# chanchanchan97/ICAFusion

Measured on AMD Instinct MI355X. Metric: RGB/IR image-pairs/sec (two-stream forward + NMS), higher is better.
Workload: dtype bf16

## Files before the change

icafusion_amd/csrc/conv_common.h:

```cpp
#pragma once
#include "icaf_common.h"

namespace icaf {

struct ConvP {
    const void* x; const void* w; const float* bias; void* y; const void* res;
    long long x_gs, w_gs, bias_gs, y_gs, res_gs;
    int B, H, W, Cin, ldx, Ho, Wo, Cout, ldy, kh, kw, sh, sw, ph, pw, ldr, Kp, act;
    int M, K, nchunks, mtiles, ntiles;
    int vec_y, vec_r;
    unsigned int x_bytes, w_bytes;
    float alpha_acc[2], alpha_res[2];
    const float* pre; int pre_h, pre_w, ldpre, pre_mode;
    const void* w1; const float* bias1;
    long long w1_gs, bias1_gs; int Kp1; unsigned int w1_bytes;
    const void* w2; const float* bias2; void* y2;
    long long w2_gs, bias2_gs, y2_gs; int Kp2, Cout2, ldy2, vec_y2, keep1; unsigned int w2_bytes;
    const void* x2; long long x2_gs; int ldx2;
};

constexpr int ROWB = 64;
constexpr int ROWS = 80;
constexpr int NTHREADS = 256;

int ctile_conv_check(const icaf_conv_args* a, const ConvP& p, int shape);
int launch_ctile(const icaf_conv_args* a, const ConvP& p, int shape, hipStream_t s);
const char* ctile_tag(int shape);
int stream_check(const icaf_conv_args* a, const ConvP& p, int shape);
int launch_stream(const icaf_conv_args* a, const ConvP& p, int shape, hipStream_t s);
const char* stream_tag(int shape);
int wreg_check(const icaf_conv_args* a, const ConvP& p, int shape);
int launch_wreg(const icaf_conv_args* a, const ConvP& p, int shape, hipStream_t s);
const char* wreg_tag(int shape);
int cstream_check(const icaf_conv_args* a, const ConvP& p, int shape);
int launch_cstream(const icaf_conv_args* a, const ConvP& p, int shape, hipStream_t s);
const char* cstream_tag(int shape);
int cwide_check(const icaf_conv_args* a, const ConvP& p, int shape);
int launch_cwide(const icaf_conv_args* a, const ConvP& p, int shape, hipStream_t s);
const char* cwide_tag(int shape);
int launch_bneck(const icaf_conv_args* a, const ConvP& p, int shape, hipStream_t s);

constexpr int ACT_RELU_RES = 16 + ICAF_ACT_RELU;
template <int ACT, int DT = ICAF_F32> __device__ __forceinline__ float apply_act(float v) {
    if constexpr (ACT == ICAF_ACT_SILU) return silu_f(v);
    else if constexpr (ACT == ICAF_ACT_GELU) return DT == ICAF_F32 ? gelu_f(v) : gelu_fast_f(v);
    else if constexpr (ACT == ICAF_ACT_RELU || ACT == ACT_RELU_RES) return fmaxf(v, 0.0f);
    else return v;
}
template <int DT> __device__ __forceinline__ void load_res_quad(const typename Elem<DT>::type* __restrict__ rg, int m, int ldr, int n, int Cout, int vec_r, float (&r)[4]) {
    using E = Elem<DT>;
#pragma unroll
    for (int j = 0; j < 4; ++j) r[j] = 0.0f;
    if (m < 0 || n >= Cout) return;
    const typename E::type* rp = rg + (long long)m * ldr + n;
    if (vec_r && n + 4 <= Cout) {
        if constexpr (DT == ICAF_F32) {
            const f32x4 t = *(const f32x4*)rp;
#pragma unroll
            for (int j = 0; j < 4; ++j) r[j] = t[j];
        } else {
            const u32x2 t = *(const u32x2*)rp;
            if constexpr (DT == ICAF_BF16) {
                r[0] = __uint_as_float(t[0] << 16); r[1] = __uint_as_float(t[0] & 0xffff0000u);
                r[2] = __uint_as_float(t[1] << 16); r[3] = __uint_as_float(t[1] & 0xffff0000u);
            } else {
                r[0] = f16_to_f32((unsigned short)(t[0] & 0xffffu)); r[1] = f16_to_f32((unsigned short)(t[0] >> 16));
                r[2] = f16_to_f32((unsigned short)(t[1] & 0xffffu)); r[3] = f16_to_f32((unsigned short)(t[1] >> 16));
            }
        }
    } else {
        for (int j = 0; j < 4 && n + j < Cout; ++j) r[j] = E::ld(rp + j);
    }
}
template <int ACT, int DT = ICAF_F32> __device__ __forceinline__ void apply_act4(const float (&x)[4], float (&y)[4]) {
    if constexpr (ACT == ICAF_ACT_SILU) silu4_f(x, y);
    else {
#pragma unroll
        for (int j = 0; j < 4; ++j) y[j] = apply_act<ACT, DT>(x[j]);
    }
}

__device__ __forceinline__ int xcd_tile(int ntile_total) {
    const int bid = blockIdx.x, q = ntile_total >> 3, r = ntile_total & 7, xcd = bid & 7, idx = bid >> 3;
    return (xcd < r ? xcd * (q + 1) : r * (q + 1) + (xcd - r) * q) + idx;
}

template <int DT, int ODT, int BM, int BN, int WM, int WN, int ACT, bool PRE, bool SECOND = false, bool WB = false, bool FULLVEC = false, typename RowMap>
__device__ __forceinline__ void epilogue(f32x16 (&acc)[WN / 32][WM / 32], unsigned char* lds, const ConvP& p, int g, RowMap row_to_m, int n0) {
    using E = Elem<DT>;
    using EO = Elem<ODT>;
    constexpr int TM = WM / 32, TN = WN / 32;
    constexpr int WAVES_M = BM / WM;
    constexpr int NT = (BM / WM) * (BN / WN) * 64;
    constexpr int VO = 16 / EO::BYTES;
    constexpr int SO = BN * EO::BYTES + 16;
    const int tid = threadIdx.x, lane = tid & 63, wave = tid >> 6, l31 = lane & 31, hi = lane >> 5;
    const int wm = wave % WAVES_M, wn = wave / WAVES_M;
    const float alpha_acc = SECOND ? 1.0f : p.alpha_acc[g], alpha_res = p.alpha_res[g];
    const float* __restrict__ bias = SECOND ? (p.bias2 ? p.bias2 + g * p.bias2_gs : nullptr) : (p.bias ? p.bias + g * p.bias_gs : nullptr);
    const int Cout = SECOND ? p.Cout2 : p.Cout, ldy = SECOND ? p.ldy2 : p.ldy, vec_y = SECOND ? p.vec_y2 : p.vec_y;
    static_assert(ACT != ACT_RELU_RES || (!PRE && !SECOND && !WB && !FULLVEC && ODT == DT), "res_mode = 1: a plain same-type layer");
    if constexpr (PRE) {
        constexpr int SOF = BN * 4 + 16;
#pragma unroll
        for (int a = 0; a < TN; ++a) {
            f32x4 bq[4];
#pragma unroll
            for (int q = 0; q < 4; ++q) {
                const int n = n0 + wn * WN + a * 32 + 8 * q + 4 * hi;
                const bool okn = bias && n < Cout;
                const float* bp = okn ? bias + n : (const float*)p.w;
                const f32x4 t = *(const f32x4*)bp;
                bq[q] = okn ? t : f32x4{0.f, 0.f, 0.f, 0.f};
            }
#pragma unroll
            for (int q = 0; q < 4; ++q) {
                const int nl = wn * WN + a * 32 + 8 * q + 4 * hi;
#pragma unroll
                for (int b = 0; b < TM; ++b) {
                    const int ml = wm * WM + b * 32 + l31;
                    f32x4 t;
#pragma unroll
                    for (int j = 0; j < 4; ++j) t[j] = acc[a][b][4 * q + j] + bq[q][j];
                    *(f32x4*)(lds + ml * SOF + nl * 4) = t;
                }
            }
        }
        __syncthreads();
        typename EO::type* __restrict__ yg2 = SECOND ? (typename EO::type*)p.y2 + g * p.y2_gs : (typename EO::type*)p.y + g * p.y_gs;
        const typename E::type* __restrict__ rg2 = (!SECOND && p.res) ? (const typename E::type*)p.res + g * p.res_gs : nullptr;
        constexpr int VPR2 = BN / VO, NVEC2 = BM * VPR2, NIT2 = (NVEC2 + NT - 1) / NT;
        const float sy = (float)p.pre_h / (float)p.Ho, sx = (float)p.pre_w / (float)p.Wo;
#pragma unroll 2
        for (int it = 0; it < NIT2; ++it) {
            const int idx = tid + it * NT;
            if (idx >= NVEC2) break;
            const int row = idx / VPR2, cv = idx - row * VPR2;
            const int m = row_to_m(row), n = n0 + cv * VO;
            if (m < 0 || n >= Cout) continue;
            const float* pt4[4];
            float lx, ly;
            {
#pragma clang fp contract(off)
                const int wo = m % p.Wo, t = m / p.Wo, ho = t % p.Ho, bi = t / p.Ho;
                float fy = ((float)ho + 0.5f) * sy - 0.5f, fx = ((float)wo + 0.5f) * sx - 0.5f;
                fy = fy < 0.0f ? 0.0f : fy;
                fx = fx < 0.0f ? 0.0f : fx;
                int y0 = (int)fy, x0 = (int)fx;
                y0 = y0 < p.pre_h - 1 ? y0 : p.pre_h - 1;
                x0 = x0 < p.pre_w - 1 ? x0 : p.pre_w - 1;
                int y1 = y0 < p.pre_h - 1 ? y0 + 1 : y0, x1 = x0 < p.pre_w - 1 ? x0 + 1 : x0;
                ly = fy - (float)y0;
                lx = fx - (float)x0;
                if (p.pre_mode == 1) {
                    y0 = y1 = (int)((long long)ho * p.pre_h / p.Ho);
                    x0 = x1 = (int)((long long)wo * p.pre_w / p.Wo);
                    ly = lx = 0.0f;
                }
                const float* base = p.pre + (long long)bi * p.pre_h * p.pre_w * p.ldpre + n;
                pt4[0] = base + (long long)(y0 * p.pre_w + x0) * p.ldpre;
                pt4[1] = base + (long long)(y0 * p.pre_w + x1) * p.ldpre;
                pt4[2] = base + (long long)(y1 * p.pre_w + x0) * p.ldpre;
                pt4[3] = base + (long long)(y1 * p.pre_w + x1) * p.ldpre;
            }
            const int nvalid = (Cout - n) < VO ? (Cout - n) : VO;
            float v[VO];
#pragma unroll
            for (int k4 = 0; k4 < VO / 4; ++k4) {
                const f32x4 t = *(const f32x4*)(lds + row * SOF + (cv * VO + 4 * k4) * 4);
                float pv[4] = {0.f, 0.f, 0.f, 0.f};
                if (n + 4 * k4 < Cout) {
                    const f32x4 t00 = *(const f32x4*)(pt4[0] + 4 * k4), t01 = *(const f32x4*)(pt4[1] + 4 * k4);
                    const f32x4 t10 = *(const f32x4*)(pt4[2] + 4 * k4), t11 = *(const f32x4*)(pt4[3] + 4 * k4);
                    {
#pragma clang fp contract(off)
                        const float wx0 = 1.0f - lx, wy0 = 1.0f - ly;
#pragma unroll
                        for (int j = 0; j < 4; ++j) {
                            const float top = t00[j] * wx0 + t01[j] * lx;
                            const float bot = t10[j] * wx0 + t11[j] * lx;
                            pv[j] = top * wy0 + bot * ly;
                        }
                    }
                }
#pragma unroll
                for (int j = 0; j < 4; ++j) v[4 * k4 + j] = apply_act<ACT, DT>(t[j] + pv[j]) * alpha_acc;
            }
            u32x4 o = pack16<ODT>(v);
            typename EO::type* yp = yg2 + (long long)m * ldy + n;
            if (rg2) {
                unpack16<ODT>(o, v);
                const typename E::type* rp = rg2 + (long long)m * p.ldr + n;
                for (int j = 0; j < nvalid; ++j) v[j] = __builtin_fmaf(alpha_res, E::ld(rp + j), v[j]);
                o = pack16<ODT>(v);
            }
            if (vec_y && nvalid == VO) *(u32x4*)yp = o;
            else {
                unpack16<ODT>(o, v);
                for (int j = 0; j < nvalid; ++j) EO::st(yp + j, v[j]);
            }
        }
        return;
    }
#pragma unroll
    for (int a = 0; a < TN; ++a) {
        f32x4 bq[4];
#pragma unroll
        for (int q = 0; q < 4; ++q) {
            const int n = n0 + wn * WN + a * 32 + 8 * q + 4 * hi;
            const bool okn = bias && n < Cout;
            const float* bp = okn ? bias + n : (const float*)p.w;
            const f32x4 t = *(const f32x4*)bp;
            bq[q] = okn ? t : f32x4{0.f, 0.f, 0.f, 0.f};
        }
#pragma unroll
        for (int q = 0; q < 4; ++q) {
            const int nl = wn * WN + a * 32 + 8 * q + 4 * hi;
            const float bv[4] = {bq[q][0], bq[q][1], bq[q][2], bq[q][3]};
#pragma unroll
            for (int b = 0; b < TM; ++b) {
                const int ml = wm * WM + b * 32 + l31;
                float v[4], xin[4];
#pragma unroll
                for (int j = 0; j < 4; ++j) xin[j] = acc[a][b][4 * q + j] + bv[j] + 0.0f;
                if constexpr (ACT == ACT_RELU_RES) {
                    float rq[4];
                    load_res_quad<DT>((const typename E::type*)p.res + g * p.res_gs, row_to_m(ml), p.ldr, n0 + nl, Cout, p.vec_r, rq);
#pragma unroll
                    for (int j = 0; j < 4; ++j) xin[j] += rq[j];
                }
                apply_act4<ACT, DT>(xin, v);
#pragma unroll
                for (int j = 0; j < 4; ++j) v[j] *= alpha_acc;
                unsigned char* dst = lds + ml * SO + nl * EO::BYTES;
                if constexpr (EO::BYTES == 4) {
                    *(f32x4*)dst = f32x4{v[0], v[1], v[2], v[3]};
                } else {
                    u32x2 pk;
                    if constexpr (ODT == ICAF_BF16) { pk[0] = pack2_bf16(v[0], v[1]); pk[1] = pack2_bf16(v[2], v[3]); }
                    else { pk[0] = pack2_f16(v[0], v[1]); pk[1] = pack2_f16(v[2], v[3]); }
                    *(u32x2*)dst = pk;
                }
            }
        }
    }
    __syncthreads();

    typename EO::type* __restrict__ yg = SECOND ? (typename EO::type*)p.y2 + g * p.y2_gs : (typename EO::type*)p.y + g * p.y_gs;
    const typename E::type* __restrict__ rg = (!SECOND && p.res && ACT != ACT_RELU_RES) ? (const typename E::type*)p.res + g * p.res_gs : nullptr;
    constexpr int VPR = BN / VO;
    constexpr int NVEC = BM * VPR;
    constexpr int NIT = (NVEC + NT - 1) / NT;
    if constexpr (FULLVEC) {
        static_assert(!WB && NVEC % NT == 0 && (VPR & (VPR - 1)) == 0, "whole rounds of power-of-two rows");
#pragma unroll
        for (int it = 0; it < NIT; ++it) {
            const int idx = tid + it * NT, row = idx / VPR, cv = idx & (VPR - 1);
            const int m = row_to_m(row);
            if (m >= 0) *(u32x4*)(yg + (long long)m * ldy + n0 + cv * VO) = *(const u32x4*)(lds + row * SO + cv * 16);
        }
        return;
    }
    if constexpr (VO == E::VEC && NVEC % NT == 0 && (VPR & (VPR - 1)) == 0) {
        if (vec_y && n0 + BN <= Cout && (!rg || p.vec_r)) {
            if (!rg) {
#pragma unroll
                for (int it = 0; it < NIT; ++it) {
                    const int idx = tid + it * NT, row = idx / VPR, cv = idx & (VPR - 1);
                    const int m = row_to_m(row);
// ... 174 lines not shown
```

icafusion_amd/csrc/dmff.hip:

```cpp
#include <cstdlib>
#include "icaf_common.h"
#include "attn_core.h"

namespace icaf {

static inline unsigned grid_for(long long total) {
    long long b = (total + 255) / 256;
    if (b > 256 * 16) b = 256 * 16;
    if (b < 1) b = 1;
    return (unsigned)b;
}

struct PoolDiv { FastDiv nv, N, tw; };
template <int DT, bool I32>
__global__ __launch_bounds__(256) void pool_tokens_kernel(const typename Elem<DT>::type* __restrict__ f0, int ld0,
                                                          const typename Elem<DT>::type* __restrict__ f1, int ld1,
                                                          const float* __restrict__ pos0, const float* __restrict__ pos1,
                                                          typename Elem<DT>::type* __restrict__ tok, int B, int H, int W, int C, int th,
                                                          int tw, int kh, int kw, int sh, int sw, float w1_0, float w2_0, float w1_1,
                                                          float w2_1, PoolDiv dv) {
    using E = Elem<DT>;
    const int nv = C / E::VEC, N = th * tw;
    const long long per_g = (long long)B * N * nv, total = 2 * per_g;
    const float inv_area = 1.0f / (float)(kh * kw);
    for (long long idx = (long long)blockIdx.x * blockDim.x + threadIdx.x; idx < total; idx += (long long)gridDim.x * blockDim.x) {
        const int g = idx >= per_g;
        const long long r = idx - (g ? per_g : 0);
        int v, n, b, oy, ox;
        if constexpr (I32) {
            unsigned int bn, uv, un, ub, uoy, uox;
            fd_divmod((unsigned int)r, dv.nv, bn, uv);
            fd_divmod(bn, dv.N, ub, un);
            fd_divmod(un, dv.tw, uoy, uox);
            v = (int)uv; n = (int)un; b = (int)ub; oy = (int)uoy; ox = (int)uox;
        } else {
            v = (int)(r % nv);
            const long long bn = r / nv;
            n = (int)(bn % N); b = (int)(bn / N);
            oy = n / tw; ox = n - oy * tw;
        }
        const typename E::type* f = g ? f1 : f0;
        const int ld = g ? ld1 : ld0;
        float sum[E::VEC], mx[E::VEC];
#pragma unroll
        for (int j = 0; j < E::VEC; ++j) { sum[j] = 0.0f; mx[j] = -INFINITY; }
        const typename E::type* f00 = f + (((long long)b * H + oy * sh) * W + ox * sw) * ld + v * E::VEC;
        for (int dy = 0; dy < kh; ++dy) {
            const typename E::type* frow = f00 + (long long)dy * W * ld;
            for (int dx0 = 0; dx0 < kw; dx0 += 4) {
                u32x4 raw[4];
#pragma unroll
                for (int u = 0; u < 4; ++u)
                    if (dx0 + u < kw) raw[u] = *(const u32x4*)(frow + (long long)(dx0 + u) * ld);
#pragma unroll
                for (int u = 0; u < 4; ++u) {
                    if (dx0 + u < kw) {
                        float t[E::VEC];
                        unpack16<DT>(raw[u], t);
#pragma unroll
                        for (int j = 0; j < E::VEC; ++j) { sum[j] += t[j]; mx[j] = fmaxf(mx[j], t[j]); }
                    }
                }
            }
        }
        const float w1 = g ? w1_1 : w1_0, w2 = g ? w2_1 : w2_0;
        const float* pos = (g ? pos1 : pos0) + (long long)n * C + v * E::VEC;
        float o[E::VEC];
#pragma unroll
        for (int j = 0; j < E::VEC; ++j) o[j] = (sum[j] * inv_area) * w1 + mx[j] * w2 + pos[j];
        *(u32x4*)(tok + (((long long)g * B + b) * N + n) * C + v * E::VEC) = pack16<DT>(o);
    }
}

template <int DT, int R, int TR>
__global__ __launch_bounds__(1024) void pool_tokens_rows_kernel(const typename Elem<DT>::type* __restrict__ f0, int ld0,
                                                                const typename Elem<DT>::type* __restrict__ f1, int ld1,
                                                                const float* __restrict__ pos0, const float* __restrict__ pos1,
                                                                typename Elem<DT>::type* __restrict__ tok, int B, int H, int W, int C,
                                                                int th, int tw, int kh, int kw, int sh, int sw, float w1_0, float w2_0,
                                                                float w1_1, float w2_1) {
    using E = Elem<DT>;
    constexpr int V = E::VEC;
    extern __shared__ __attribute__((aligned(16))) unsigned char lds_raw[];
    const int nv = C / V, nitem = W * nv;
    float* csum = (float*)lds_raw;
    u32x4* cmax = (u32x4*)(csum + (size_t)TR * nitem * V);
    const int nblk = gridDim.x, bid = blockIdx.x;
    const int qd = nblk >> 3, rm = nblk & 7, xcd = bid & 7, ix = bid >> 3;
    const int row = (xcd < rm ? xcd * (qd + 1) : rm * (qd + 1) + (xcd - rm) * qd) + ix;
    const int thb = (th + TR - 1) / TR;
    const int g = row / (B * thb), r = row - g * (B * thb), b = r / thb, oy0 = (r - b * thb) * TR;
    const int ntr = th - oy0 < TR ? th - oy0 : TR;
    const int nrow = kh + (ntr - 1) * sh;
    const typename E::type* f = g ? f1 : f0;
    const int ld = g ? ld1 : ld0;
    const typename E::type* frow = f + ((long long)b * H + oy0 * sh) * W * ld;
    const long long rstride = (long long)W * ld;
    for (int item = threadIdx.x; item < nitem; item += blockDim.x) {
        const int x = item / nv, v = item - x * nv;
        const typename E::type* p0 = frow + (long long)x * ld + v * V;
        float sum[TR][V], mx[TR][V];
#pragma unroll
        for (int t = 0; t < TR; ++t)
#pragma unroll
            for (int j = 0; j < V; ++j) { sum[t][j] = 0.0f; mx[t][j] = -INFINITY; }
        for (int d0 = 0; d0 < nrow; d0 += R) {
            u32x4 raw[R];
#pragma unroll
            for (int u = 0; u < R; ++u) {
                const int d = d0 + u < nrow ? d0 + u : nrow - 1;
                raw[u] = *(const u32x4*)(p0 + d * rstride);
            }
#pragma unroll
            for (int u = 0; u < R; ++u) {
                float t[V];
                unpack16<DT>(raw[u], t);
#pragma unroll
                for (int k = 0; k < TR; ++k) {
                    const int dd = d0 + u - k * sh;
                    if (dd >= 0 && dd < kh && k < ntr) {
                        asm volatile("");
#pragma unroll
                        for (int j = 0; j < V; ++j) {
                            sum[k][j] += t[j];
                            mx[k][j] = fmaxf(mx[k][j], t[j]);
                        }
                    }
                }
            }
        }
#pragma unroll
        for (int k = 0; k < TR; ++k) {
#pragma unroll
            for (int j = 0; j < V; j += 4)
                *(f32x4*)(csum + ((size_t)k * nitem + item) * V + j) = f32x4{sum[k][j], sum[k][j + 1], sum[k][j + 2], sum[k][j + 3]};
            cmax[(size_t)k * nitem + item] = pack16<DT>(mx[k]);
        }
    }
    __syncthreads();
    const float inv_area = 1.0f / (float)(kh * kw);
    const float w1 = g ? w1_1 : w1_0, w2 = g ? w2_1 : w2_0;
    const int N = th * tw, per = tw * nv;
    for (int o = threadIdx.x; o < ntr * per; o += blockDim.x) {
        const int k = o / per, o1 = o - k * per, ox = o1 / nv, v = o1 - ox * nv;
        float sum[V], mx[V];
#pragma unroll
        for (int j = 0; j < V; ++j) { sum[j] = 0.0f; mx[j] = -INFINITY; }
        for (int dx = 0; dx < kw; ++dx) {
            const size_t it = (size_t)k * nitem + (size_t)(ox * sw + dx) * nv + v;
            float m[V];
            unpack16<DT>(cmax[it], m);
#pragma unroll
            for (int j = 0; j < V; j += 4) {
                const f32x4 a = *(const f32x4*)(csum + it * V + j);
#pragma unroll
                for (int e = 0; e < 4; ++e) { sum[j + e] += a[e]; mx[j + e] = fmaxf(mx[j + e], m[j + e]); }
            }
        }
        const int n = (oy0 + k) * tw + ox;
        const float* pos = (g ? pos1 : pos0) + (long long)n * C + v * V;
        float out[V];
#pragma unroll
        for (int j = 0; j < V; ++j) out[j] = (sum[j] * inv_area) * w1 + mx[j] * w2 + pos[j];
        *(u32x4*)(tok + (((long long)g * B + b) * N + n) * C + v * V) = pack16<DT>(out);
    }
}

template <int DT>
__global__ __launch_bounds__(256) void layernorm_kernel(const typename Elem<DT>::type* __restrict__ x, typename Elem<DT>::type* __restrict__ y,
                                                        const float* __restrict__ g0, const float* __restrict__ b0,
                                                        const float* __restrict__ g1, const float* __restrict__ b1,
                                                        long long rows_per_group, int C, int groups, float eps) {
    using E = Elem<DT>;
    constexpr int MAXV = 4;
    const int lane = threadIdx.x & 63;
    const long long row = (long long)blockIdx.x * (blockDim.x >> 6) + (threadIdx.x >> 6);
    if (row >= rows_per_group * groups) return;
    const int grp = (int)(row / rows_per_group);
    const float* gam = grp ? g1 : g0;
    const float* bet = grp ? b1 : b0;
    const int nv = C / E::VEC;
    float val[MAXV][E::VEC];
    float s = 0.0f;
#pragma unroll
    for (int i = 0; i < MAXV; ++i) {
        const int v = lane + 64 * i;
        if (v < nv) {
            unpack16<DT>(*(const u32x4*)(x + row * C + v * E::VEC), val[i]);
#pragma unroll
            for (int j = 0; j < E::VEC; ++j) s += val[i][j];
        }
    }
#pragma unroll
    for (int o = 32; o > 0; o >>= 1) s += __shfl_xor(s, o);
    const float mean = s / (float)C;
    float q = 0.0f;
#pragma unroll
    for (int i = 0; i < MAXV; ++i) {
        const int v = lane + 64 * i;
        if (v < nv) {
#pragma unroll
            for (int j = 0; j < E::VEC; ++j) { const float d = val[i][j] - mean; q += d * d; }
        }
    }
#pragma unroll
    for (int o = 32; o > 0; o >>= 1) q += __shfl_xor(q, o);
    const float rstd = 1.0f / sqrtf(q / (float)C + eps);
#pragma unroll
    for (int i = 0; i < MAXV; ++i) {
        const int v = lane + 64 * i;
        if (v < nv) {
            float o[E::VEC];
#pragma unroll
            for (int j = 0; j < E::VEC; ++j) o[j] = (val[i][j] - mean) * rstd * gam[v * E::VEC + j] + bet[v * E::VEC + j];
            *(u32x4*)(y + row * C + v * E::VEC) = pack16<DT>(o);
        }
    }
}

template <int DT, int MAXV>
__device__ __forceinline__ void layernorm_row(const typename Elem<DT>::type* __restrict__ x, typename Elem<DT>::type* __restrict__ y,
                                              const float* __restrict__ g0, const float* __restrict__ b0,
                                              const float* __restrict__ g1, const float* __restrict__ b1,
                                              long long rows_per_group, int C, int groups, float eps) {
    using E = Elem<DT>;
    const int lane = threadIdx.x & 63;
    const long long row = (long long)blockIdx.x * (blockDim.x >> 6) + (threadIdx.x >> 6);
    if (row >= rows_per_group * groups) return;
    const int grp = (int)(row / rows_per_group);
    const float* gam = grp ? g1 : g0;
    const float* bet = grp ? b1 : b0;
    const int nv = C / E::VEC;
    float val[MAXV][E::VEC];
    float s = 0.0f;
#pragma unroll
    for (int i = 0; i < MAXV; ++i) {
        const int v = lane + 64 * i;
        if (v < nv) {
            unpack16<DT>(*(const u32x4*)(x + row * C + v * E::VEC), val[i]);
#pragma unroll
            for (int j = 0; j < E::VEC; ++j) s += val[i][j];
        }
    }
#pragma unroll
    for (int o = 32; o > 0; o >>= 1) s += __shfl_xor(s, o);
    const float mean = s / (float)C;
// ... 490 lines not shown
    ICAF_HIP(hipGetDevice(&dev));
    if (lds > 64 * 1024 && dev >= 0 && dev < ICAF_MAX_DEVICES && !attr_set[dev]) {
        ICAF_HIP(hipFuncSetAttribute((const void*)cross_attn_kernel<DT, DKP>, hipFuncAttributeMaxDynamicSharedMemorySize, 160 * 1024));
        attr_set[dev] = true;
    }
    const float scale_l2e = (float)((1.0 / sqrt((double)DK)) * 1.4426950408889634);
    dim3 grid((unsigned)qsplit, (unsigned)heads, (unsigned)(2 * B));
    if (c.remap) grid = dim3((unsigned)(qsplit * heads * 2 * B), 1u, 1u);
    hipLaunchKernelGGL((cross_attn_kernel<DT, DKP>), grid, dim3(256), lds, s, (const T*)qkv, (T*)out, B, N, C, DK, NP, scale_l2e, c.remap ? qsplit : 0);
    ICAF_LAUNCH_CHECK();
    return ICAF_OK;
}

template <int DT>
static int dispatch_attn(const void* qkv, void* out, int B, int N, int C, int heads, const AttnCfg& c, hipStream_t s) {
    switch (c.dkp) {
        case 16: return launch_attn<DT, 16>(qkv, out, B, N, C, heads, c, s);
        case 32: return launch_attn<DT, 32>(qkv, out, B, N, C, heads, c, s);
        case 48: return launch_attn<DT, 48>(qkv, out, B, N, C, heads, c, s);
        case 64: return launch_attn<DT, 64>(qkv, out, B, N, C, heads, c, s);
        case 96: return launch_attn<DT, 96>(qkv, out, B, N, C, heads, c, s);
        default: return launch_attn<DT, 128>(qkv, out, B, N, C, heads, c, s);
    }
}

struct PoolCfg { int kernel, R, TR, index64; size_t row_lds; };

static int pool_select(int dtype, int B, int H, int W, int C, int th, int tw, int kh, int kw, int sh, int sw, PoolCfg& c) {
    if (dtype < ICAF_F32 || dtype > ICAF_F16) return fail(ICAF_ERR_ARG, "bad dtype %d", dtype);
    const int vec = dtype == ICAF_F32 ? 4 : 8;
    if (C < 1 || C % vec) return fail(ICAF_ERR_ARG, "icaf_dmff_pool_tokens: C/ld must be multiples of %d", vec);
    if (B < 1 || th < 1 || tw < 1 || sh < 1 || sw < 1) return fail(ICAF_ERR_ARG, "icaf_dmff_pool_tokens: bad B / token grid / stride");
    if ((th - 1) * sh + kh > H || (tw - 1) * sw + kw > W || kh < 1 || kw < 1) return fail(ICAF_ERR_ARG, "icaf_dmff_pool_tokens: window exceeds the feature map");
    c.row_lds = (size_t)W * (C / vec) * (vec * sizeof(float) + 16);
    c.kernel = 0; c.R = 0; c.TR = 0; c.index64 = 0;
    if ((kh > sh || kw > sw) && c.row_lds <= 160 * 1024) {
        c.TR = (2 * c.row_lds <= 160 * 1024 && kh > sh && kh + sh <= 12 && 2 * B * ((th + 1) / 2) >= 256) ? 2 : 1;
        const int nrow = kh + (c.TR - 1) * sh;
        c.R = nrow <= 4 ? 4 : nrow <= 8 ? 8 : 12;
        c.kernel = 1;
        return ICAF_OK;
    }
    const long long total = 2LL * B * th * tw * (C / vec);
    c.index64 = total >= (1ll << 31) || g_opt.index64 != 0;
    return ICAF_OK;
}

}

using namespace icaf;

namespace {
template <int DT>
int run_pool_tokens(const void* f0, int ld0, const void* f1, int ld1, const float* p0, const float* p1, void* tok, int B, int H, int W, int C,
                    int th, int tw, int kh, int kw, int sh, int sw, float a0, float b0, float a1, float b1, const PoolCfg& c, hipStream_t s) {
    using T = typename Elem<DT>::type;
    if (c.kernel == 1) {
        const int tr = c.TR, rsel = c.R == 4 ? 0 : c.R == 8 ? 1 : 2;
        const size_t rows_lds = tr * c.row_lds;
        static size_t attr_bytes[ICAF_MAX_DEVICES][3][2] = {};
        int dev = 0;
        ICAF_HIP(hipGetDevice(&dev));
        const void* fns[3][2] = {{(const void*)pool_tokens_rows_kernel<DT, 4, 1>, (const void*)pool_tokens_rows_kernel<DT, 4, 2>},
                                 {(const void*)pool_tokens_rows_kernel<DT, 8, 1>, (const void*)pool_tokens_rows_kernel<DT, 8, 2>},
                                 {(const void*)pool_tokens_rows_kernel<DT, 12, 1>, (const void*)pool_tokens_rows_kernel<DT, 12, 2>}};
        const void* fn = fns[rsel][tr - 1];
        if (rows_lds > 64 * 1024 && dev >= 0 && dev < ICAF_MAX_DEVICES && rows_lds > attr_bytes[dev][rsel][tr - 1]) {
            ICAF_HIP(hipFuncSetAttribute(fn, hipFuncAttributeMaxDynamicSharedMemorySize, (int)rows_lds));
            attr_bytes[dev][rsel][tr - 1] = rows_lds;
        }
        const dim3 grid((unsigned)(2 * B * ((th + tr - 1) / tr))), block(1024);
#define ICAF_POOL_ROWS(RR, TT)                                                                                                              \
    pool_tokens_rows_kernel<DT, RR, TT><<<grid, block, rows_lds, s>>>((const T*)f0, ld0, (const T*)f1, ld1, p0, p1, (T*)tok, B, H, W, C, th, tw, \
                                                                      kh, kw, sh, sw, a0, b0, a1, b1)
        if (rsel == 0) { if (tr == 2) ICAF_POOL_ROWS(4, 2); else ICAF_POOL_ROWS(4, 1); }
        else if (rsel == 1) { if (tr == 2) ICAF_POOL_ROWS(8, 2); else ICAF_POOL_ROWS(8, 1); }
        else { if (tr == 2) ICAF_POOL_ROWS(12, 2); else ICAF_POOL_ROWS(12, 1); }
#undef ICAF_POOL_ROWS
        ICAF_LAUNCH_CHECK();
        return ICAF_OK;
    }
    const long long total = 2LL * B * th * tw * (C / Elem<DT>::VEC);
    const PoolDiv dv{make_fastdiv((unsigned)(C / Elem<DT>::VEC)), make_fastdiv((unsigned)(th * tw)), make_fastdiv((unsigned)tw)};
    if (!c.index64)
        pool_tokens_kernel<DT, true><<<dim3(grid_for(total)), dim3(256), 0, s>>>((const T*)f0, ld0, (const T*)f1, ld1, p0, p1, (T*)tok, B, H, W, C,
                                                                                  th, tw, kh, kw, sh, sw, a0, b0, a1, b1, dv);
    else
        pool_tokens_kernel<DT, false><<<dim3(grid_for(total)), dim3(256), 0, s>>>((const T*)f0, ld0, (const T*)f1, ld1, p0, p1, (T*)tok, B, H, W, C,
                                                                                   th, tw, kh, kw, sh, sw, a0, b0, a1, b1, dv);
    ICAF_LAUNCH_CHECK();
    return ICAF_OK;
}
template <int DT>
int run_layernorm(const void* x, void* y, const float* g0, const float* b0, const float* g1, const float* b1, long long rpg, int C, int groups,
                  float eps, hipStream_t s) {
    using T = typename Elem<DT>::type;
    const long long rows = rpg * groups;
    layernorm_kernel<DT><<<dim3((unsigned)((rows + 3) / 4)), dim3(256), 0, s>>>((const T*)x, (T*)y, g0, b0, g1, b1, rpg, C, groups, eps);
    ICAF_LAUNCH_CHECK();
    return ICAF_OK;
}
template <int DT>
int run_upsample_merge(const void* tok, const void* f0, int ld0, const void* f1, int ld1, void* out, int ldo, int B, int H, int W, int C, int th,
                       int tw, hipStream_t s) {
    using T = typename Elem<DT>::type;
    const long long total = 2LL * B * H * W * (C / Elem<DT>::VEC);
    upsample_merge_kernel<DT><<<dim3(grid_for(total)), dim3(256), 0, s>>>((const T*)tok, (const T*)f0, ld0, (const T*)f1, ld1, (T*)out, ldo, B,
                                                                           H, W, C, th, tw);
    ICAF_LAUNCH_CHECK();
    return ICAF_OK;
}
}

#define DISPATCH_DT(dtype, FN, ...)                                  \
    switch (dtype) {                                                 \
        case ICAF_F32: return FN<ICAF_F32>(__VA_ARGS__);             \
        case ICAF_BF16: return FN<ICAF_BF16>(__VA_ARGS__);           \
        case ICAF_F16: return FN<ICAF_F16>(__VA_ARGS__);             \
        default: return fail(ICAF_ERR_ARG, "bad dtype %d", dtype);   \
    }

extern "C" int icaf_dmff_pool_tokens(const void* fea_rgb, int ld_rgb, const void* fea_ir, int ld_ir, const float* pos_rgb,
                                     const float* pos_ir, void* tokens, int dtype, int B, int H, int W, int C, int th, int tw, int kh,
                                     int kw, int sh, int sw, float w1_rgb, float w2_rgb, float w1_ir, float w2_ir, icaf_stream_t s) {
    if (!fea_rgb || !fea_ir || !pos_rgb || !pos_ir || !tokens) return fail(ICAF_ERR_ARG, "icaf_dmff_pool_tokens: null pointer");
    const int vec = dtype == ICAF_F32 ? 4 : 8;
    if (C % vec || ld_rgb % vec || ld_ir % vec) return fail(ICAF_ERR_ARG, "icaf_dmff_pool_tokens: C/ld must be multiples of %d", vec);
    PoolCfg c;
    if (const int st = pool_select(dtype, B, H, W, C, th, tw, kh, kw, sh, sw, c)) return st;
    DISPATCH_DT(dtype, run_pool_tokens, fea_rgb, ld_rgb, fea_ir, ld_ir, pos_rgb, pos_ir, tokens, B, H, W, C, th, tw, kh, kw, sh, sw, w1_rgb,
                w2_rgb, w1_ir, w2_ir, c, S(s));
}

extern "C" int icaf_dmff_pool_config(int dtype, int B, int H, int W, int C, int th, int tw, int kh, int kw, int sh, int sw, int* kernel, int* R,
                                     int* TR, int* index64) {
    if (!kernel || !R || !TR || !index64) return fail(ICAF_ERR_ARG, "icaf_dmff_pool_config: null pointer");
    PoolCfg c;
    if (const int st = pool_select(dtype, B, H, W, C, th, tw, kh, kw, sh, sw, c)) return st;
    *kernel = c.kernel;
    *R = c.R;
    *TR = c.TR;
    *index64 = c.index64;
    return ICAF_OK;
}

extern "C" int icaf_layernorm(const void* x, void* y, const float* gamma0, const float* beta0, const float* gamma1, const float* beta1,
                              int dtype, long long rows_per_group, int C, int groups, float eps, icaf_stream_t s) {
    if (!x || !y || !gamma0 || !beta0) return fail(ICAF_ERR_ARG, "icaf_layernorm: null pointer");
    if (groups < 1 || groups > 2 || (groups == 2 && (!gamma1 || !beta1))) return fail(ICAF_ERR_ARG, "icaf_layernorm: bad groups");
    const int vec = dtype == ICAF_F32 ? 4 : 8;
    if (C % vec || C > 2048) return fail(ICAF_ERR_ARG, "icaf_layernorm: C=%d must be a multiple of %d and <= 2048", C, vec);
    if (C > 64 * 4 * vec)
        return layernorm_wide_dispatch(x, y, gamma0, beta0, gamma1 ? gamma1 : gamma0, beta1 ? beta1 : beta0, rows_per_group, C, groups, eps, S(s));
    DISPATCH_DT(dtype, run_layernorm, x, y, gamma0, beta0, gamma1 ? gamma1 : gamma0, beta1 ? beta1 : beta0, rows_per_group, C, groups, eps, S(s));
}

extern "C" int icaf_cross_attention(const void* qkv, void* out, int dtype, int B, int N, int C, int heads, icaf_stream_t s) {
    if (!qkv || !out) return fail(ICAF_ERR_ARG, "icaf_cross_attention: null pointer");
    AttnCfg c;
    if (const int st = attn_select(dtype, B, N, C, heads, c)) return st;
    if (c.form) return attn_stream_dispatch(dtype, qkv, out, B, N, C, heads, c, S(s));
    DISPATCH_DT(dtype, dispatch_attn, qkv, out, B, N, C, heads, c, S(s));
}

extern "C" int icaf_cross_attention_config(int dtype, int B, int N, int C, int heads, int* dkp, int* qsplit, int* remap) {
    if (!dkp || !qsplit || !remap) return fail(ICAF_ERR_ARG, "icaf_cross_attention_config: null pointer");
    AttnCfg c;
    if (const int st = attn_select(dtype, B, N, C, heads, c)) return st;
    *dkp = c.dkp;
    *qsplit = c.qsplit;
    *remap = c.remap;
    return ICAF_OK;
// ... 60 lines not shown
```

icafusion_amd/csrc/igemm.hip:

```cpp
#include "conv_common.h"

static_assert(sizeof(icaf_conv_args) == 312, "icaf_conv_args layout is mirrored by ctypes in icafusion_amd/_lib.py");
static_assert(sizeof(icaf_bneck_args) == 376, "icaf_bneck_args layout is mirrored by ctypes in icafusion_amd/_lib.py");

namespace icaf {

template <int DT, int ODT, int BM, int BN, int WM, int WN, int ACT, int RB, int NS, int MODE, bool PRE, bool CHAIN = false>
__global__ __launch_bounds__((BM / WM) * (BN / WN) * 64) void igemm_dma_kernel(const ConvP p) {
    using E = Elem<DT>;
    using L = TileLds<DT, ODT, BM, BN>;
    constexpr int VEC = E::VEC;
    constexpr int BK = RB / E::BYTES;
    constexpr int SPR = RB / 16;
    constexpr int RPI = 1024 / RB;
    constexpr int AI = BM / RPI, BI = BN / RPI;
    constexpr int NW = (BM / WM) * (BN / WN);
    constexpr int NA = AI / NW;
    constexpr int NBF = BI / NW, NBR = BI % NW;
    constexpr int NBMAX = NBF + (NBR ? 1 : 0);
    constexpr int TM = WM / 32, TN = WN / 32;
    constexpr int WAVES_M = BM / WM;
    constexpr int STAGE = (BM + BN) * RB;
    constexpr int NSTEP = RB / 32;
    static_assert(AI % NW == 0 && (NW == 4 || NW == 8), "tile shape");
// ... 509 lines not shown
    void (*name)(const ConvFamily&, const icaf_conv_args*, int shape, char* buf, int len);
    const char* prefix;
    const char* (*tag)(int shape);
};
static const char* const kTypeName[] = {"f32", "bf16", "f16"};
static bool whole_range(int) { return true; }
static void shape_name(const ConvFamily& f, const icaf_conv_args* a, int shape, char* buf, int len) {
    snprintf(buf, len, "%s_%s_%s", f.prefix, kTypeName[a->dtype], f.tag(shape));
}
static void igemm_name(const ConvFamily&, const icaf_conv_args* a, int id, char* buf, int len) {
    snprintf(buf, len, "igemm%s_%s_%s_%s", kPipes[id / 10].tag, kTypeName[a->dtype], kTypeName[a->out_dtype], kTiles[id % 10 - 1].tag);
}
static const ConvFamily kFamilies[] = {
    {1, 34, 0, igemm_built, igemm_check, launch_igemm_any, igemm_name, nullptr, nullptr},
    {41, 45, 40, whole_range, ctile_conv_check, launch_ctile, shape_name, "ctile", ctile_tag},
    {51, 52, 50, whole_range, stream_check, launch_stream, shape_name, "igemm_stream", stream_tag},
    {61, 66, 60, whole_range, wreg_check, launch_wreg, shape_name, "igemm_wreg", wreg_tag},
    {71, 71, 70, whole_range, cstream_check, launch_cstream, shape_name, "cstream", cstream_tag},
    {81, 85, 80, whole_range, cwide_check, launch_cwide, shape_name, "cwide", cwide_tag},
};

static const ConvFamily* family_of(int id) {
    for (const ConvFamily& f : kFamilies)
        if (id >= f.lo && id <= f.hi && f.built(id)) return &f;
    return nullptr;
}

static int pick_tile(const icaf_conv_args* a, const ConvP& p) {
    const bool dma_ok = p.x_bytes != 0;
    if (a->tile) return (a->tile < 40 && a->tile % 10 <= 4 && !dma_ok) ? a->tile % 10 + 10 : a->tile;
    if (a->x2) return 81;
    const bool f32 = a->dtype == ICAF_F32 || a->out_dtype == ICAF_F32;
    const int N = a->Cout;
    const long long M = p.M;
    auto blocks = [&](int t) { return ((M + kTiles[t - 1].bm - 1) / kTiles[t - 1].bm) * ((N + kTiles[t - 1].bn - 1) / kTiles[t - 1].bn) * a->groups; };
    int t;
    if (N > 64 && !f32) t = 1;
    else if (N > 32) t = 2;
    else t = 3;
    if (t == 1 && blocks(1) < 512 && blocks(2) > blocks(1)) t = 2;
    if (blocks(t) < 512 && blocks(4) > blocks(t)) t = 4;
    if (!dma_ok) return t + 10;
    const int eb = a->dtype == ICAF_F32 ? 4 : 2;
    if (a->w2) {
        const int c = a->Cout > a->Cout2 ? a->Cout : a->Cout2;
        const bool w128 = ((long long)a->Cin * eb) % 128 == 0;
        if (c <= 64) return w128 ? 22 : 2;
        return w128 ? 21 : 1;
    }
    if (a->pre) {
        if (t > 2) t = 2;
        return ((long long)a->Cin * eb) % 128 == 0 ? t + 20 : t;
    }
    return (long long)p.K * eb >= 256 ? t + 20 : t;
}

static int validate(const icaf_conv_args* a) {
    if (!a || !a->x || !a->w || !a->y) return fail(ICAF_ERR_ARG, "icaf_conv2d: null pointer");
    if (a->groups < 1 || a->groups > 2) return fail(ICAF_ERR_ARG, "icaf_conv2d: groups must be 1 or 2");
    if (a->tile != 0 && !family_of(a->tile)) return fail(ICAF_ERR_ARG, "icaf_conv2d: unknown launch configuration %d", a->tile);
    const int vec = a->dtype == ICAF_F32 ? 4 : 8;
    if (a->dtype < 0 || a->dtype > 2) return fail(ICAF_ERR_ARG, "icaf_conv2d: bad dtype %d", a->dtype);
    if (a->out_dtype != a->dtype && a->out_dtype != ICAF_F32) return fail(ICAF_ERR_ARG, "icaf_conv2d: out_dtype must equal dtype or be fp32");
    if (a->Cin % vec || a->ldx % vec) return fail(ICAF_ERR_ARG, "icaf_conv2d: Cin (%d) and ldx (%d) must be multiples of %d", a->Cin, a->ldx, vec);
    if (((uintptr_t)a->x & 15) || ((uintptr_t)a->w & 15)) return fail(ICAF_ERR_ARG, "icaf_conv2d: x / w must be 16-byte aligned");
    if (a->B < 1 || a->Ho < 1 || a->Wo < 1 || a->Cout < 1 || a->kh < 1 || a->kw < 1 || a->sh < 1 || a->sw < 1)
        return fail(ICAF_ERR_ARG, "icaf_conv2d: bad geometry");
    if (a->Ho != (a->H + 2 * a->ph - a->kh) / a->sh + 1 || a->Wo != (a->W + 2 * a->pw - a->kw) / a->sw + 1)
        return fail(ICAF_ERR_ARG, "icaf_conv2d: output size does not match input/kernel/stride/padding");
    const int ka = a->dtype == ICAF_F32 ? 32 : 64;
    if (a->Kp % ka || a->Kp < a->kh * a->kw * a->Cin) return fail(ICAF_ERR_ARG, "icaf_conv2d: Kp=%d must be a multiple of %d covering K=%d", a->Kp, ka, a->kh * a->kw * a->Cin);
    if (a->act < 0 || a->act > ICAF_ACT_RELU) return fail(ICAF_ERR_ARG, "icaf_conv2d: bad activation code %d", a->act);
    if (a->res_mode < 0 || a->res_mode > 1) return fail(ICAF_ERR_ARG, "icaf_conv2d: res_mode must be 0 (residual behind the activation) or 1 (in front of it), got %d", a->res_mode);
    if (a->ldy < a->Cout) return fail(ICAF_ERR_ARG, "icaf_conv2d: ldy < Cout");
    if (a->res && a->ldr < a->Cout) return fail(ICAF_ERR_ARG, "icaf_conv2d: ldr < Cout");
    if ((long long)a->B * a->Ho * a->Wo > 0x7fffffffLL) return fail(ICAF_ERR_ARG, "icaf_conv2d: too many output pixels");
    if (a->w2 && (!a->y2 || a->Cout2 < 1 || a->ldy2 < a->Cout2 || a->Kp2 < a->Cout || (a->Kp2 * (a->dtype == ICAF_F32 ? 4 : 2)) % 128 || ((uintptr_t)a->w2 & 15)))
        return fail(ICAF_ERR_ARG, "icaf_conv2d: chained 1x1 needs y2, ldy2 >= Cout2 >= 1, Kp2 >= Cout in whole 128-byte slices, aligned w2");
    if (a->x2 && (!a->w2 || a->dtype == ICAF_F32 || a->Kp2 < 2 * a->Cout || a->ldx2 < a->Cout))
        return fail(ICAF_ERR_ARG, "icaf_conv2d: x2 (the second half of the chained 1x1's input) needs w2, a 16-bit type, Kp2 >= 2 Cout and ldx2 >= Cout");
    if (a->pre && (a->pre_mode < 0 || a->pre_mode > 1)) return fail(ICAF_ERR_ARG, "icaf_conv2d: pre_mode must be 0 (bilinear) or 1 (nearest)");
    if (a->pre && (a->pre_h < 1 || a->pre_w < 1 || a->ldpre < a->Cout || (a->ldpre & 3) || ((uintptr_t)a->pre & 15) || a->groups != 1))
        return fail(ICAF_ERR_ARG, "icaf_conv2d: pre needs pre_h, pre_w >= 1, ldpre >= Cout and a multiple of 4, 16-byte alignment, groups == 1");
    return ICAF_OK;
}

static void fill(const icaf_conv_args* a, ConvP& p) {
    p.x = a->x; p.w = a->w; p.bias = a->bias; p.y = a->y; p.res = a->res;
    p.x_gs = a->x_gs; p.w_gs = a->w_gs; p.bias_gs = a->bias_gs; p.y_gs = a->y_gs; p.res_gs = a->res_gs;
    p.B = a->B; p.H = a->H; p.W = a->W; p.Cin = a->Cin; p.ldx = a->ldx; p.Ho = a->Ho; p.Wo = a->Wo; p.Cout = a->Cout;
    p.ldy = a->ldy; p.kh = a->kh; p.kw = a->kw; p.sh = a->sh; p.sw = a->sw; p.ph = a->ph; p.pw = a->pw; p.ldr = a->ldr;
    p.Kp = a->Kp; p.act = a->act;
    p.x2 = a->x2; p.x2_gs = a->x2_gs; p.ldx2 = a->ldx2;
    p.M = a->B * a->Ho * a->Wo;
    p.K = a->kh * a->kw * a->Cin;
    const int bk = a->dtype == ICAF_F32 ? 16 : 32;
    p.nchunks = (p.K + bk - 1) / bk;
    p.mtiles = p.ntiles = 0;
    const int vo = a->out_dtype == ICAF_F32 ? 4 : 8, vi = a->dtype == ICAF_F32 ? 4 : 8;
    const int yb = a->out_dtype == ICAF_F32 ? 4 : 2, eb = a->dtype == ICAF_F32 ? 4 : 2;
    p.vec_y = (a->ldy % vo == 0) && (((uintptr_t)a->y & 15) == 0) && ((a->y_gs * yb) % 16 == 0);
    p.vec_r = a->res && (a->ldr % vi == 0) && (((uintptr_t)a->res & 15) == 0) && ((a->res_gs * eb) % 16 == 0);
    const long long xb = (((long long)a->B * a->H * a->W - 1) * a->ldx + a->Cin) * eb;
    const long long np = ((long long)a->Cout + 127) / 128 * 128;
    const long long wb = np * a->Kp * eb;
    if (xb < 0x7fffff00LL && wb < 0x7fffff00LL) { p.x_bytes = (unsigned)xb; p.w_bytes = (unsigned)wb; }
    else { p.x_bytes = 0; p.w_bytes = 0; }
    for (int i = 0; i < 2; ++i) { p.alpha_acc[i] = a->alpha_acc[i]; p.alpha_res[i] = a->alpha_res[i]; }
    p.pre = a->pre; p.pre_h = a->pre_h; p.pre_w = a->pre_w; p.ldpre = a->ldpre; p.pre_mode = a->pre_mode;
    p.w1 = nullptr; p.bias1 = nullptr; p.w1_gs = p.bias1_gs = 0; p.Kp1 = 0; p.w1_bytes = 0;
    p.w2 = a->w2; p.bias2 = a->bias2; p.y2 = a->y2; p.w2_gs = a->w2_gs; p.bias2_gs = a->bias2_gs; p.y2_gs = a->y2_gs;
    p.Kp2 = a->Kp2; p.Cout2 = a->Cout2; p.ldy2 = a->ldy2; p.keep1 = a->chain_keep;
    p.vec_y2 = a->w2 && (a->ldy2 % vo == 0) && (((uintptr_t)a->y2 & 15) == 0) && ((a->y2_gs * yb) % 16 == 0);
    p.w2_bytes = a->w2 ? (unsigned)((((long long)a->Cout2 + 127) / 128 * 128) * a->Kp2 * eb) : 0;
}

int conv_prepare(const icaf_conv_args* a, ConvP& p) {
    int st = validate(a);
    if (st) return st;
    fill(a, p);
    return ICAF_OK;
}

static int resolve(const icaf_conv_args* a, ConvP& p, const ConvFamily*& f, int& shape) {
    int st = conv_prepare(a, p);
    if (st) return st;
    if (a->res_mode == 1 && (!a->res || a->act != ICAF_ACT_RELU || a->alpha_acc[0] != 1.0f || a->alpha_acc[1] != 1.0f || a->alpha_res[0] != 1.0f ||
                             a->alpha_res[1] != 1.0f || a->pre || a->w2 || a->x2 || a->out_dtype != a->dtype))
        return fail(ICAF_ERR_UNSUPPORTED, "icaf_conv2d: res_mode = 1 needs a residual, ACT_RELU, alpha_acc = alpha_res = 1, no pre term, no chained layer "
                                          "and out_dtype == dtype");
    const int id = pick_tile(a, p);
    if (a->x2 && id != 81 && id != 82) return fail(ICAF_ERR_UNSUPPORTED, "icaf_conv2d: x2 (C3 tail) is built for launch configurations 81 / 82 only (tile %d)", id);
    f = family_of(id);
    if (!f) return fail(ICAF_ERR_ARG, "icaf_conv2d: unknown launch configuration %d", id);
    shape = id - f->base;
    return f->check(a, p, shape);
}

}

using namespace icaf;

extern "C" int icaf_conv2d(const icaf_conv_args* a, icaf_stream_t s) {
    ConvP p;
    const ConvFamily* f;
    int shape;
    const int st = resolve(a, p, f, shape);
    return st ? st : f->launch(a, p, shape, S(s));
}

extern "C" int icaf_conv2d_kernel_name(const icaf_conv_args* a, char* buf, int buf_len) {
    ConvP p;
    const ConvFamily* f;
    int shape;
    const int st = resolve(a, p, f, shape);
    if (st) return st;
    f->name(*f, a, shape, buf, buf_len);
    return ICAF_OK;
}

extern "C" int icaf_conv2d_config_ids(int* ids, int cap) {
    int n = 0;
    for (const ConvFamily& f : kFamilies)
        for (int id = f.lo; id <= f.hi; ++id)
            if (family_of(id)) {
                if (ids && n < cap) ids[n] = id;
// ... 24 lines not shown
```

Baseline: 16750.

## Precompute bilinear tap table in LDS and templatize pool-token tap span

The conv epilogue that adds an upsampled 'pre' map now computes the bilinear source offset, neighbour flags and weights once per output row and stores them in LDS. Previously this index and weight work was redone for every vector of the row. The pool-tokens kernel now loads a whole pooling window, or one row of it, in a single unrolled batch sized 4, 8 or 16 at compile time, replacing the fixed groups of four per row. The changes add LDS use beyond the staging area, more kernel instantiations and a 32-bit offset limit that the validator enforces.

```diff
diff --git a/icafusion_amd/csrc/conv_common.h b/icafusion_amd/csrc/conv_common.h
--- a/icafusion_amd/csrc/conv_common.h
+++ b/icafusion_amd/csrc/conv_common.h
@@ -102,6 +102,36 @@
     static_assert(ACT != ACT_RELU_RES || (!PRE && !SECOND && !WB && !FULLVEC && ODT == DT), "res_mode = 1: a plain same-type layer");
     if constexpr (PRE) {
         constexpr int SOF = BN * 4 + 16;
+        constexpr int TAB = BN * 4;
+        auto tap_table = [&]() {
+            const float sy = (float)p.pre_h / (float)p.Ho, sx = (float)p.pre_w / (float)p.Wo;
+            for (int row = tid; row < BM; row += NT) {
+                const int m = row_to_m(row);
+                u32x4 e = {0u, 0u, 0u, 0u};
+                if (m >= 0) {
+#pragma clang fp contract(off)
+                    const int wo = m % p.Wo, t = m / p.Wo, ho = t % p.Ho, bi = t / p.Ho;
+                    float fy = ((float)ho + 0.5f) * sy - 0.5f, fx = ((float)wo + 0.5f) * sx - 0.5f;
+                    fy = fy < 0.0f ? 0.0f : fy;
+                    fx = fx < 0.0f ? 0.0f : fx;
+                    int y0 = (int)fy, x0 = (int)fx;
+                    y0 = y0 < p.pre_h - 1 ? y0 : p.pre_h - 1;
+                    x0 = x0 < p.pre_w - 1 ? x0 : p.pre_w - 1;
+                    int y1 = y0 < p.pre_h - 1 ? y0 + 1 : y0, x1 = x0 < p.pre_w - 1 ? x0 + 1 : x0;
+                    float ly = fy - (float)y0, lx = fx - (float)x0;
+                    if (p.pre_mode == 1) {
+                        y0 = y1 = (int)((long long)ho * p.pre_h / p.Ho);
+                        x0 = x1 = (int)((long long)wo * p.pre_w / p.Wo);
+                        ly = lx = 0.0f;
+                    }
+                    e[0] = (unsigned)(((bi * p.pre_h + y0) * p.pre_w + x0) * p.ldpre);
+                    e[1] = (x1 != x0 ? 1u : 0u) | (y1 != y0 ? 2u : 0u);
+                    e[2] = __float_as_uint(lx);
+                    e[3] = __float_as_uint(ly);
+                }
+                *(u32x4*)(lds + row * SOF + TAB) = e;
+            }
+        };
 #pragma unroll
         for (int a = 0; a < TN; ++a) {
             f32x4 bq[4];
@@ -126,11 +156,12 @@
                 }
             }
         }
+        tap_table();
         __syncthreads();
         typename EO::type* __restrict__ yg2 = SECOND ? (typename EO::type*)p.y2 + g * p.y2_gs : (typename EO::type*)p.y + g * p.y_gs;
         const typename E::type* __restrict__ rg2 = (!SECOND && p.res) ? (const typename E::type*)p.res + g * p.res_gs : nullptr;
         constexpr int VPR2 = BN / VO, NVEC2 = BM * VPR2, NIT2 = (NVEC2 + NT - 1) / NT;
-        const float sy = (float)p.pre_h / (float)p.Ho, sx = (float)p.pre_w / (float)p.Wo;
+        const int xstep = p.ldpre, ystep = p.pre_w * p.ldpre;
 #pragma unroll 2
         for (int it = 0; it < NIT2; ++it) {
             const int idx = tid + it * NT;
@@ -138,31 +169,14 @@
             const int row = idx / VPR2, cv = idx - row * VPR2;
             const int m = row_to_m(row), n = n0 + cv * VO;
             if (m < 0 || n >= Cout) continue;
+            const u32x4 e = *(const u32x4*)(lds + row * SOF + TAB);
+            const float lx = __uint_as_float(e[2]), ly = __uint_as_float(e[3]);
+            const int dx = (e[1] & 1u) ? xstep : 0, dy = (e[1] & 2u) ? ystep : 0;
             const float* pt4[4];
-            float lx, ly;
-            {
-#pragma clang fp contract(off)
-                const int wo = m % p.Wo, t = m / p.Wo, ho = t % p.Ho, bi = t / p.Ho;
-                float fy = ((float)ho + 0.5f) * sy - 0.5f, fx = ((float)wo + 0.5f) * sx - 0.5f;
-                fy = fy < 0.0f ? 0.0f : fy;
-                fx = fx < 0.0f ? 0.0f : fx;
-                int y0 = (int)fy, x0 = (int)fx;
-                y0 = y0 < p.pre_h - 1 ? y0 : p.pre_h - 1;
-                x0 = x0 < p.pre_w - 1 ? x0 : p.pre_w - 1;
-                int y1 = y0 < p.pre_h - 1 ? y0 + 1 : y0, x1 = x0 < p.pre_w - 1 ? x0 + 1 : x0;
-                ly = fy - (float)y0;
-                lx = fx - (float)x0;
-                if (p.pre_mode == 1) {
-                    y0 = y1 = (int)((long long)ho * p.pre_h / p.Ho);
-                    x0 = x1 = (int)((long long)wo * p.pre_w / p.Wo);
-                    ly = lx = 0.0f;
-                }
-                const float* base = p.pre + (long long)bi * p.pre_h * p.pre_w * p.ldpre + n;
-                pt4[0] = base + (long long)(y0 * p.pre_w + x0) * p.ldpre;
-                pt4[1] = base + (long long)(y0 * p.pre_w + x1) * p.ldpre;
-                pt4[2] = base + (long long)(y1 * p.pre_w + x0) * p.ldpre;
-                pt4[3] = base + (long long)(y1 * p.pre_w + x1) * p.ldpre;
-            }
+            pt4[0] = p.pre + ((int)e[0] + n);
+            pt4[1] = pt4[0] + dx;
+            pt4[2] = pt4[0] + dy;
+            pt4[3] = pt4[2] + dx;
             const int nvalid = (Cout - n) < VO ? (Cout - n) : VO;
             float v[VO];
 #pragma unroll
@@ -183,8 +197,12 @@
                         }
                     }
                 }
-#pragma unroll
-                for (int j = 0; j < 4; ++j) v[4 * k4 + j] = apply_act<ACT, DT>(t[j] + pv[j]) * alpha_acc;
+                float xin[4], av[4];
+#pragma unroll
+                for (int j = 0; j < 4; ++j) xin[j] = t[j] + pv[j];
+                apply_act4<ACT, DT>(xin, av);
+#pragma unroll
+                for (int j = 0; j < 4; ++j) v[4 * k4 + j] = av[j] * alpha_acc;
             }
             u32x4 o = pack16<ODT>(v);
             typename EO::type* yp = yg2 + (long long)m * ldy + n;
diff --git a/icafusion_amd/csrc/dmff.hip b/icafusion_amd/csrc/dmff.hip
--- a/icafusion_amd/csrc/dmff.hip
+++ b/icafusion_amd/csrc/dmff.hip
@@ -12,7 +12,37 @@
 }
 
 struct PoolDiv { FastDiv nv, N, tw; };
-template <int DT, bool I32>
+__device__ __forceinline__ float pool_mix(float sum, float mx, float inv_area, float w1, float w2, float pos) {
+    return (sum * inv_area) * w1 + mx * w2 + pos;
+}
+template <int DT, int NB>
+__device__ __forceinline__ void pool_span(const typename Elem<DT>::type* start, long long rstride, int ld, int kw, int n,
+                                          float (&sum)[Elem<DT>::VEC], float (&mx)[Elem<DT>::VEC]) {
+    using E = Elem<DT>;
+    u32x4 raw[NB];
+    long long row = 0, off = 0;
+    int dx = 0;
+#pragma unroll
+    for (int u = 0; u < NB; ++u) {
+        raw[u] = *(const u32x4*)(start + off);
+        if (u + 1 < n) {
+            ++dx;
+            off += ld;
+            if (dx == kw) { dx = 0; row += rstride; off = row; }
+        }
+    }
+#pragma unroll
+    for (int u = 0; u < NB; ++u) {
+        if (u < n) {
+            asm volatile("");
+            float t[E::VEC];
+            unpack16<DT>(raw[u], t);
+#pragma unroll
+            for (int j = 0; j < E::VEC; ++j) { sum[j] += t[j]; mx[j] = fmaxf(mx[j], t[j]); }
+        }
+    }
+}
+template <int DT, bool I32, int NB>
 __global__ __launch_bounds__(256) void pool_tokens_kernel(const typename Elem<DT>::type* __restrict__ f0, int ld0,
                                                           const typename Elem<DT>::type* __restrict__ f1, int ld1,
                                                           const float* __restrict__ pos0, const float* __restrict__ pos1,
@@ -45,29 +75,19 @@
 #pragma unroll
         for (int j = 0; j < E::VEC; ++j) { sum[j] = 0.0f; mx[j] = -INFINITY; }
         const typename E::type* f00 = f + (((long long)b * H + oy * sh) * W + ox * sw) * ld + v * E::VEC;
-        for (int dy = 0; dy < kh; ++dy) {
-            const typename E::type* frow = f00 + (long long)dy * W * ld;
-            for (int dx0 = 0; dx0 < kw; dx0 += 4) {
-                u32x4 raw[4];
-#pragma unroll
-                for (int u = 0; u < 4; ++u)
-                    if (dx0 + u < kw) raw[u] = *(const u32x4*)(frow + (long long)(dx0 + u) * ld);
-#pragma unroll
-                for (int u = 0; u < 4; ++u) {
-                    if (dx0 + u < kw) {
-                        float t[E::VEC];
-                        unpack16<DT>(raw[u], t);
-#pragma unroll
-                        for (int j = 0; j < E::VEC; ++j) { sum[j] += t[j]; mx[j] = fmaxf(mx[j], t[j]); }
-                    }
-                }
-            }
+        const long long rstride = (long long)W * ld;
+        const bool whole = kh <= NB && kw <= NB && kh * kw <= NB;
+        const int nrows = whole ? 1 : kh, rowtaps = whole ? kh * kw : kw;
+        for (int dy = 0; dy < nrows; ++dy) {
+            const typename E::type* frow = f00 + dy * rstride;
+            for (int dx0 = 0; dx0 < rowtaps; dx0 += NB)
+                pool_span<DT, NB>(frow + (long long)dx0 * ld, rstride, ld, kw, rowtaps - dx0 < NB ? rowtaps - dx0 : NB, sum, mx);
         }
         const float w1 = g ? w1_1 : w1_0, w2 = g ? w2_1 : w2_0;
         const float* pos = (g ? pos1 : pos0) + (long long)n * C + v * E::VEC;
         float o[E::VEC];
 #pragma unroll
-        for (int j = 0; j < E::VEC; ++j) o[j] = (sum[j] * inv_area) * w1 + mx[j] * w2 + pos[j];
+        for (int j = 0; j < E::VEC; ++j) o[j] = pool_mix(sum[j], mx[j], inv_area, w1, w2, pos[j]);
         *(u32x4*)(tok + (((long long)g * B + b) * N + n) * C + v * E::VEC) = pack16<DT>(o);
     }
 }
@@ -161,7 +181,7 @@
         const float* pos = (g ? pos1 : pos0) + (long long)n * C + v * V;
         float out[V];
 #pragma unroll
-        for (int j = 0; j < V; ++j) out[j] = (sum[j] * inv_area) * w1 + mx[j] * w2 + pos[j];
+        for (int j = 0; j < V; ++j) out[j] = pool_mix(sum[j], mx[j], inv_area, w1, w2, pos[j]);
         *(u32x4*)(tok + (((long long)g * B + b) * N + n) * C + v * V) = pack16<DT>(out);
     }
 }
@@ -818,12 +838,14 @@
     }
     const long long total = 2LL * B * th * tw * (C / Elem<DT>::VEC);
     const PoolDiv dv{make_fastdiv((unsigned)(C / Elem<DT>::VEC)), make_fastdiv((unsigned)(th * tw)), make_fastdiv((unsigned)tw)};
-    if (!c.index64)
-        pool_tokens_kernel<DT, true><<<dim3(grid_for(total)), dim3(256), 0, s>>>((const T*)f0, ld0, (const T*)f1, ld1, p0, p1, (T*)tok, B, H, W, C,
-                                                                                  th, tw, kh, kw, sh, sw, a0, b0, a1, b1, dv);
-    else
-        pool_tokens_kernel<DT, false><<<dim3(grid_for(total)), dim3(256), 0, s>>>((const T*)f0, ld0, (const T*)f1, ld1, p0, p1, (T*)tok, B, H, W, C,
-                                                                                   th, tw, kh, kw, sh, sw, a0, b0, a1, b1, dv);
+    const long long ntap = (long long)kh * kw;
+    const int span = ntap <= 16 ? (int)ntap : kw, nb = span <= 4 ? 4 : span <= 8 ? 8 : 16;
+#define ICAF_POOL_ELEM(I32, NB)                                                                                                             \
+    pool_tokens_kernel<DT, I32, NB><<<dim3(grid_for(total)), dim3(256), 0, s>>>((const T*)f0, ld0, (const T*)f1, ld1, p0, p1, (T*)tok, B, H, W, C, \
+                                                                                 th, tw, kh, kw, sh, sw, a0, b0, a1, b1, dv)
+    if (!c.index64) { if (nb == 4) ICAF_POOL_ELEM(true, 4); else if (nb == 8) ICAF_POOL_ELEM(true, 8); else ICAF_POOL_ELEM(true, 16); }
+    else { if (nb == 4) ICAF_POOL_ELEM(false, 4); else if (nb == 8) ICAF_POOL_ELEM(false, 8); else ICAF_POOL_ELEM(false, 16); }
+#undef ICAF_POOL_ELEM
     ICAF_LAUNCH_CHECK();
     return ICAF_OK;
 }
diff --git a/icafusion_amd/csrc/igemm.hip b/icafusion_amd/csrc/igemm.hip
--- a/icafusion_amd/csrc/igemm.hip
+++ b/icafusion_amd/csrc/igemm.hip
@@ -615,6 +615,12 @@
     if (a->pre && (a->pre_mode < 0 || a->pre_mode > 1)) return fail(ICAF_ERR_ARG, "icaf_conv2d: pre_mode must be 0 (bilinear) or 1 (nearest)");
     if (a->pre && (a->pre_h < 1 || a->pre_w < 1 || a->ldpre < a->Cout || (a->ldpre & 3) || ((uintptr_t)a->pre & 15) || a->groups != 1))
         return fail(ICAF_ERR_ARG, "icaf_conv2d: pre needs pre_h, pre_w >= 1, ldpre >= Cout and a multiple of 4, 16-byte alignment, groups == 1");
+    if (a->pre) {
+        long long n = (long long)a->pre_h * a->pre_w;
+        if (n <= 0x7fffffffLL) n *= a->B;
+        if (n <= 0x7fffffffLL) n *= a->ldpre;
+        if (n > 0x7fffffffLL) return fail(ICAF_ERR_UNSUPPORTED, "icaf_conv2d: pre map of B x pre_h x pre_w x ldpre = %d x %d x %d x %d: 2^31 elements or more are not addressed", a->B, a->pre_h, a->pre_w, a->ldpre);
+    }
     return ICAF_OK;
 }
 
```

Result: no change. 16730 (-0.2%).
